# uingei/hevc

Hardware: AMD Instinct MI355X
Metric: encoded 1080p30 frames/sec/GPU; PSNR-Y parity vs libx265 at matched bitrate (higher is better)
Workload: dtype u8; 1 GPU; 1920x1080@30 SDR 8-bit Main, crf 19 capped by VBV maxrate 2940 kbps / bufsize 3528 kbit (the reference's libx265 operating point), 300-frame synthetic 'motion' clip per GPU, keyint 90 (4 closed GOPs of equal length), IPPP, full-search +-15, one clip per GPU, input resident in HBM

## Files before the change

### hevc_amd/csrc/kernels/common.h

```cpp
#pragma once
#include <stdint.h>

#if defined(__HIPCC__)
#include <hip/hip_runtime.h>
#define DEV __device__ __forceinline__
#define HD __host__ __device__
#define HDI __host__ __device__ inline
#define DEVCONST __device__ const
#define MIHEVC_GPU 1
#else
#define DEV inline
#define HD
#define HDI inline
#define DEVCONST static const
#define MIHEVC_GPU 0
#endif

#include "../../../include/mihevc.h"

namespace mihevc {

constexpr int CTU = 32;
constexpr int CTU_LOG2 = 5;
constexpr int PAD_Y = 80;
// ... 58 lines not shown
        for (int n = 0; n < 32; n++) {
            int a = (k * (2 * n + 1)) % 128;
            if (a > 64) a = 128 - a;
            t.mat[k][n] = (int8_t)(a > 32 ? -c64[64 - a] : c64[a]);
        }
    const int d[4][4] = {{29, 55, 74, 84}, {74, 74, 0, -74}, {84, -29, -74, 55}, {55, -84, 74, -29}};
    for (int i = 0; i < 4; i++) for (int j = 0; j < 4; j++) t.dst4[i][j] = (int8_t)d[i][j];
    const int lt[4][8] = {{0, 0, 0, 64, 0, 0, 0, 0}, {-1, 4, -10, 58, 17, -5, 1, 0}, {-1, 4, -11, 40, 40, -11, 4, -1}, {0, 1, -5, 17, 58, -10, 4, -1}};
    for (int i = 0; i < 4; i++) for (int j = 0; j < 8; j++) t.luma_tap[i][j] = (int8_t)lt[i][j];
    const int ct[8][4] = {{0, 64, 0, 0}, {-2, 58, 10, -2}, {-4, 54, 16, -2}, {-6, 46, 28, -4}, {-4, 36, 36, -4}, {-4, 28, 46, -6}, {-2, 16, 54, -4}, {-2, 10, 58, -2}};
    for (int i = 0; i < 8; i++) for (int j = 0; j < 4; j++) t.chroma_tap[i][j] = (int8_t)ct[i][j];
    const int ang[35] = {0, 0, 32, 26, 21, 17, 13, 9, 5, 2, 0, -2, -5, -9, -13, -17, -21, -26, -32, -26, -21, -17, -13, -9, -5, -2, 0, 2, 5, 9, 13, 17, 21, 26, 32};
    for (int i = 0; i < 35; i++) t.intra_angle[i] = (int8_t)ang[i];
    const int inv[15] = {-4096, -1638, -910, -630, -482, -390, -315, -256, -315, -390, -482, -630, -910, -1638, -4096};
    for (int i = 0; i < 15; i++) t.inv_angle[i] = (int16_t)inv[i];
    for (int q = 0; q < 52; q++) t.beta[q] = (uint8_t)(q < 16 ? 0 : q < 29 ? q - 10 : 2 * q - 38);
    const int tcv[54] = {0, 0, 0, 0, 0, 0, 0, 0, 0, 0, 0, 0, 0, 0, 0, 0, 0, 0, 1, 1, 1, 1, 1, 1, 1, 1, 1, 2, 2, 2, 2, 3, 3, 3, 3, 4, 4, 4,
                         5, 5, 6, 6, 7, 8, 9, 10, 11, 13, 14, 16, 18, 20, 22, 24};
    for (int i = 0; i < 54; i++) t.tc[i] = (uint8_t)tcv[i];
    const int qs[6] = {26214, 23302, 20560, 18396, 16384, 14564}, ls[6] = {40, 45, 51, 57, 64, 72};
    for (int i = 0; i < 6; i++) { t.quant_scale[i] = (int16_t)qs[i]; t.level_scale[i] = (uint8_t)ls[i]; }
    const int cq[14] = {29, 30, 31, 32, 33, 33, 34, 34, 35, 35, 36, 36, 37, 37};
    for (int i = 0; i < 14; i++) t.chroma_qp[i] = (int8_t)cq[i];
    for (int ty = 0; ty < 4; ty++)
        for (int tx = 0; tx < 4; tx++) t.zorder[ty * 4 + tx] = (uint8_t)(((ty >> 1) * 2 + (tx >> 1)) * 4 + (ty & 1) * 2 + (tx & 1));
    return t;
}
DEVCONST Tables g_tab = make_tables();

DEV int iabs(int v) { return v < 0 ? -v : v; }
DEV int imin(int a, int b) { return a < b ? a : b; }
DEV int imax(int a, int b) { return a > b ? a : b; }
DEV int clip3(int lo, int hi, int v) { return v < lo ? lo : v > hi ? hi : v; }
DEV int ilog2u(unsigned v) { return 31 - __builtin_clz(v | 1); }
DEV int mvd_bits(int d)
{
    int a = iabs(d);
    return a == 0 ? 1 : a == 1 ? 3 : 3 + 2 * ilog2u((unsigned)a);
}
DEV int chroma_qp_of(int qp)
{
    int q = clip3(-12, 57, qp);
    return q < 30 ? q : q > 43 ? q - 6 : g_tab.chroma_qp[q - 30];
}
DEV int zaddr(int x, int y, int ctus_w)
{
    int bx = (x & 31) >> 2, by = (y & 31) >> 2, z = 0;
    for (int i = 0; i < 3; i++) z |= ((bx >> i) & 1) << (2 * i) | ((by >> i) & 1) << (2 * i + 1);
    return (((y >> CTU_LOG2) * ctus_w + (x >> CTU_LOG2)) << 6) | z;
}
DEV void node_geom(int node, int &x, int &y, int &log2n)
{
    if (node == 0) { x = 0; y = 0; log2n = 5; }
    else if (node < 5) { int q = node - 1; x = (q & 1) * 16; y = (q >> 1) * 16; log2n = 4; }
    else { int q = (node - 5) >> 2, s = (node - 5) & 3; x = (q & 1) * 16 + (s & 1) * 8; y = (q >> 1) * 16 + (s >> 1) * 8; log2n = 3; }
}
DEV int node_of_tile(int level, int tx, int ty)
{
    if (level == 0) return 0;
    int q = (ty >> 1) * 2 + (tx >> 1);
    return level == 1 ? 1 + q : 5 + q * 4 + (ty & 1) * 2 + (tx & 1);
}

DEV uint32_t sad_packed_u8(uint32_t a, uint32_t b, uint32_t acc)
{
#if MIHEVC_GPU
    return __builtin_amdgcn_sad_u8(a, b, acc);
#else
    for (int i = 0; i < 4; i++) acc += (uint32_t)iabs((int)((a >> (8 * i)) & 255) - (int)((b >> (8 * i)) & 255));
    return acc;
#endif
}
DEV uint32_t load_u32(const void *p)
{
    uint32_t v;
    __builtin_memcpy(&v, p, 4);
    return v;
}
DEV uint32_t pk_add16(uint32_t a, uint32_t b)
{
#if MIHEVC_GPU
    typedef short v2s __attribute__((ext_vector_type(2)));
    return __builtin_bit_cast(uint32_t, (v2s)(__builtin_bit_cast(v2s, a) + __builtin_bit_cast(v2s, b)));
#else
    return ((a + b) & 0xffffu) | (((a >> 16) + (b >> 16)) << 16);
#endif
}
DEV uint32_t pk_sub16(uint32_t a, uint32_t b)
{
#if MIHEVC_GPU
    typedef short v2s __attribute__((ext_vector_type(2)));
    return __builtin_bit_cast(uint32_t, (v2s)(__builtin_bit_cast(v2s, a) - __builtin_bit_cast(v2s, b)));
#else
    return ((a - b) & 0xffffu) | (((a >> 16) - (b >> 16)) << 16);
#endif
}
DEV uint32_t pk_max_i16(uint32_t a, uint32_t b)
{
#if MIHEVC_GPU
    uint32_t r;
    asm("v_pk_max_i16 %0, %1, %2" : "=v"(r) : "v"(a), "v"(b));
    return r;
#else
    const int al = (int16_t)(a & 0xffffu), ah = (int16_t)(a >> 16), bl = (int16_t)(b & 0xffffu), bh = (int16_t)(b >> 16);
    return (uint32_t)((al > bl ? al : bl) & 0xffff) | ((uint32_t)((ah > bh ? ah : bh) & 0xffff) << 16);
#endif
}

DEV uint32_t perm_bytes(uint32_t a, uint32_t b, uint32_t sel)
{
#if MIHEVC_GPU
    return __builtin_amdgcn_perm(a, b, sel);
#else
    const uint64_t ab = ((uint64_t)a << 32) | b;
    uint32_t r = 0;
    for (int i = 0; i < 4; i++) r |= (uint32_t)((ab >> (8 * ((sel >> (8 * i)) & 7))) & 255u) << (8 * i);
    return r;
#endif
}
DEV void transpose_bytes4(const uint32_t (&r)[4], uint32_t (&c)[4])
{
    const uint32_t t0 = perm_bytes(r[1], r[0], 0x05010400u), t1 = perm_bytes(r[1], r[0], 0x07030602u);
    const uint32_t t2 = perm_bytes(r[3], r[2], 0x05010400u), t3 = perm_bytes(r[3], r[2], 0x07030602u);
    c[0] = perm_bytes(t2, t0, 0x05040100u); c[1] = perm_bytes(t2, t0, 0x07060302u);
    c[2] = perm_bytes(t3, t1, 0x05040100u); c[3] = perm_bytes(t3, t1, 0x07060302u);
}

#if !MIHEVC_GPU
inline bool g_emu_mixed_wave = false;
#endif
DEV bool wave_all(bool p)
{
#if MIHEVC_GPU
    return __all(p) != 0;
#else
    return p && !g_emu_mixed_wave;
#endif
}

DEV uint64_t qsad_u8(uint64_t ref8, uint32_t cur, uint64_t acc)
{
#if MIHEVC_GPU
    return __builtin_amdgcn_qsad_pk_u16_u8(ref8, cur, acc);
#else
    uint64_t out = 0;
    for (int j = 0; j < 4; j++) {
        uint32_t w = (uint32_t)(ref8 >> (8 * j)), a = (uint32_t)((acc >> (16 * j)) & 0xffff);
        for (int i = 0; i < 4; i++) a += (uint32_t)iabs((int)((w >> (8 * i)) & 255) - (int)((cur >> (8 * i)) & 255));
        out |= (uint64_t)(a & 0xffff) << (16 * j);
    }
    return out;
#endif
}
DEV uint32_t align_bytes(uint32_t hi, uint32_t lo, int shift_bytes)
{
#if MIHEVC_GPU
    return __builtin_amdgcn_alignbyte(hi, lo, (uint32_t)shift_bytes);
#else
    return (uint32_t)(((((uint64_t)hi) << 32) | lo) >> (8 * shift_bytes));
#endif
}
template <typename T>
DEV void copy_window(T *lds, int ls, const T *plane, int pstride, int ox, int oy, int w, int h, int lo_x, int hi_x, int lo_y, int hi_y, int tid)
{
    constexpr int per = 4 / (int)sizeof(T);
    constexpr int CH = 6;
    const int dpr = w / per, col = tid & 31, rg = tid >> 5;
    for (int d = col; d < dpr; d += 32) {
        const int x = clip3(lo_x, hi_x - (per - 1), ox + d * per);
        for (int r0 = rg; r0 < h; r0 += CH * (NT / 32)) {
            uint32_t v[CH];
#pragma unroll
            for (int k = 0; k < CH; k++) {
                const int r = r0 + k * (NT / 32);
                if (r < h) v[k] = load_u32(plane + (ptrdiff_t)clip3(lo_y, hi_y, oy + r) * pstride + x);
            }
#pragma unroll
            for (int k = 0; k < CH; k++) {
                const int r = r0 + k * (NT / 32);
                if (r < h) __builtin_memcpy(__builtin_assume_aligned(lds + r * ls + d * per, 4), &v[k], 4);
            }
        }
    }
}

DEV int wave_uniform(int v)
{
#if MIHEVC_GPU
    v = __builtin_amdgcn_readfirstlane(v);
#endif
    return v;
}
DEV int opaque_zero()
{
    int z = 0;
#if MIHEVC_GPU
    asm volatile("" : "+v"(z));
#endif
    return z;
}
DEV uint32_t load_u32_aligned(const void *p)
{
    uint32_t v;
    __builtin_memcpy(&v, __builtin_assume_aligned(p, 4), 4);
    return v;
}
DEV void store_u32_aligned(void *p, uint32_t v) { __builtin_memcpy(__builtin_assume_aligned(p, 4), &v, 4); }
DEV void store4(uint8_t *p, int v0, int v1, int v2, int v3) { store_u32_aligned(p, (uint32_t)v0 | (uint32_t)v1 << 8 | (uint32_t)v2 << 16 | (uint32_t)v3 << 24); }
DEV void store4(uint16_t *p, int v0, int v1, int v2, int v3)
{
    store_u32_aligned(p, (uint32_t)v0 | (uint32_t)v1 << 16);
    store_u32_aligned(p + 2, (uint32_t)v2 | (uint32_t)v3 << 16);
}
DEV void store4(int16_t *p, int v0, int v1, int v2, int v3)
{
    store_u32_aligned(p, ((uint32_t)v0 & 0xffffu) | (uint32_t)v1 << 16);
    store_u32_aligned(p + 2, ((uint32_t)v2 & 0xffffu) | (uint32_t)v3 << 16);
}
DEV void load_row8(const uint8_t *base, int idx, int (&px)[8])
{
    const int off = idx & 3;
    const uint8_t *p = base + (idx - off);
    const uint32_t d0 = load_u32_aligned(p), d1 = load_u32_aligned(p + 4), d2 = load_u32_aligned(p + 8);
    const uint32_t r0 = align_bytes(d1, d0, off), r1 = align_bytes(d2, d1, off);
#pragma unroll
    for (int i = 0; i < 4; i++) { px[i] = (int)((r0 >> (8 * i)) & 255); px[4 + i] = (int)((r1 >> (8 * i)) & 255); }
}
DEV void load_row8(const uint16_t *base, int idx, int (&px)[8])
{
    const int off = idx & 1;
    const uint16_t *p = base + (idx - off);
    uint32_t d[5];
#pragma unroll
    for (int k = 0; k < 5; k++) d[k] = load_u32_aligned(p + 2 * k);
#pragma unroll
    for (int k = 0; k < 4; k++) {
        const uint32_t r = align_bytes(d[k + 1], d[k], 2 * off);
        px[2 * k] = (int)(r & 65535); px[2 * k + 1] = (int)(r >> 16);
    }
}

DEV int dot4_i8(uint32_t a, uint32_t b, int acc)
{
#if MIHEVC_GPU
    return __builtin_amdgcn_sdot4((int)a, (int)b, acc, false);
#else
    for (int i = 0; i < 4; i++) acc += (int)(int8_t)(a >> (8 * i)) * (int)(int8_t)(b >> (8 * i));
    return acc;
#endif
}
DEV int dot2_i16(uint32_t a, uint32_t b, int acc)
{
#if MIHEVC_GPU
    typedef short v2s __attribute__((ext_vector_type(2)));
    v2s va, vb;
    __builtin_memcpy(&va, &a, 4);
    __builtin_memcpy(&vb, &b, 4);
    return __builtin_amdgcn_sdot2(va, vb, acc, false);
#else
    return acc + (int)(int16_t)(a & 0xffff) * (int)(int16_t)(b & 0xffff) + (int)(int16_t)(a >> 16) * (int)(int16_t)(b >> 16);
#endif
}
DEV int dot4_i8_start(uint32_t a, uint32_t b, int start)
{
#if MIHEVC_GPU
    return __builtin_amdgcn_sdot4((int)a, (int)b, start, true);
#else
    return dot4_i8(a, b, start);
#endif
}
DEV int dot2_i16_start(uint32_t a, uint32_t b, int start)
{
#if MIHEVC_GPU
    typedef short v2s __attribute__((ext_vector_type(2)));
    v2s va, vb;
    __builtin_memcpy(&va, &a, 4);
    __builtin_memcpy(&vb, &b, 4);
    return __builtin_amdgcn_sdot2(va, vb, start, true);
#else
    return dot2_i16(a, b, start);
#endif
}

DEV uint32_t pack_lo16(int lo, int hi)
{
#if MIHEVC_GPU
    return __builtin_amdgcn_perm((uint32_t)hi, (uint32_t)lo, 0x05040100u);
#else
    return ((uint32_t)lo & 0xffffu) | ((uint32_t)hi << 16);
#endif
}

DEV void butterfly8(int (&d)[8])
{
#pragma unroll
    for (int st = 1; st < 8; st <<= 1)
#pragma unroll
        for (int i = 0; i < 8; i++)
            if (!(i & st)) { int p = d[i], q = d[i + st]; d[i] = p + q; d[i + st] = p - q; }
}
template <bool AC> DEV int hadamard8_sum(int (&m)[8][8])
{
#pragma unroll
    for (int y = 0; y < 8; y++) butterfly8(m[y]);
    int s = 0;
#pragma unroll
    for (int x = 0; x < 8; x++) {
#pragma unroll
        for (int st = 1; st < 8; st <<= 1)
#pragma unroll
            for (int i = 0; i < 8; i++)
                if (!(i & st)) { int p = m[i][x], q = m[i + st][x]; m[i][x] = p + q; m[i + st][x] = p - q; }
#pragma unroll
        for (int i = 0; i < 8; i++) if (!AC || x || i) s += iabs(m[i][x]);
    }
    return (s + 2) >> 2;
}
DEV int hadamard8_satd(int (&m)[8][8]) { return hadamard8_sum<false>(m); }
DEV int hadamard8_ac(int (&m)[8][8]) { return hadamard8_sum<true>(m); }

typedef uint32_t mfma_frag __attribute__((vector_size(16), may_alias));
typedef float mfma_acc __attribute__((vector_size(16)));
DEV float half_bits_to_float(uint32_t h)
{
#if MIHEVC_GPU && defined(__HIP_DEVICE_COMPILE__)
    const uint16_t b16 = (uint16_t)h;
    _Float16 v;
    __builtin_memcpy(&v, &b16, 2);
    return (float)v;
#else
    const uint32_t e = (h >> 10) & 31u, m = h & 1023u, b = e == 31 ? 0x7f800000u | m << 13 : (e + 112u) << 23 | m << 13;
    float f;
    __builtin_memcpy(&f, &b, 4);
    const float mag = e == 0 ? (float)(int)m * 0x1p-24f : f;
    return (h & 0x8000u) ? -mag : mag;
#endif
}
#if MIHEVC_GPU
#ifdef MIHEVC_PHASE_PROF
__device__ unsigned long long g_phase_prof[8 * 1024 * 3];
#endif
struct GpuExec {
    static DEV int lane_id()
    {
        int t = (int)threadIdx.x;
        asm volatile("" : "+v"(t));
        return t;
    }
#ifdef MIHEVC_PHASE_PROF
    template <class F> DEV void phase(F &&f, int line = __builtin_LINE(), const char *file = __builtin_FILE())
    {
        int len = 0;
// ... 140 lines not shown
```

### hevc_amd/csrc/kernels/inter.h

```cpp
#pragma once
#include "common.h"
#include "residual.h"

namespace mihevc {

template <typename T> struct InterArgs {
    Plane<const T> src[3];
    Plane<const T> ref[3];
    Plane<T> rec[3];
    int w, h, ctus_w;
    CostParams prm;
    const int16_t *centers;
    int32_t *me;
    mihevc_cu_rec *cu;
    int16_t *coef[3];
    unsigned long long *est;
    int sparse_coef;
    IpInfo *ip;
    Plane<const T> ref1[3];
    const int16_t *centers1;
    int32_t *me1;
};
template <typename T> DEV InterArgs<T> list1_view(const InterArgs<T> &a)
{
    InterArgs<T> b = a;
    for (int i = 0; i < 3; i++) b.ref[i] = a.ref1[i];
    b.centers = a.centers1; b.me = a.me1;
    return b;
}

DEVCONST int8_t kOff[9][2] = {{0, 0}, {-1, -1}, {0, -1}, {1, -1}, {-1, 0}, {1, 0}, {-1, 1}, {0, 1}, {1, 1}};
DEVCONST int8_t kRingSlot[8] = {4, 5, 2, 7, 1, 3, 6, 8};

template <typename T> struct PreArgs {
    Plane<const T> src, ref;
    uint8_t *lsrc, *lref;
    int w, h, bit_depth;
    int16_t *centers;
    unsigned *cost;
};
template <typename T> DEV void lowres_sample(const PreArgs<T> &a, int i)
{
    const int lw = a.w >> 2, n = lw * (a.h >> 2), sh = a.bit_depth - 8;
    if (i >= 2 * n) return;
    const Plane<const T> &p = i < n ? a.src : a.ref;
    const int k = i < n ? i : i - n, x = k % lw, y = k / lw;
    int s = 8 << sh;
#pragma unroll
    for (int j = 0; j < 4; j++) {
        const T *row = p.p + (ptrdiff_t)(4 * y + j) * p.stride + 4 * x;
        if (sizeof(T) == 1) {
            s = (int)sad_packed_u8(load_u32(row), 0u, (uint32_t)s);
        } else
            s += (int)row[0] + (int)row[1] + (int)row[2] + (int)row[3];
    }
    s >>= 4 + sh;
    (i < n ? a.lsrc : a.lref)[k] = (uint8_t)(s < 255 ? s : 255);
}
constexpr int PRE_SPAN = 2 * PRE_RANGE + 1;
constexpr int PRE_WIN_W = 40;
constexpr int PRE_WIN_STRIDE = 96;
struct PreShared {
    uint8_t blk[64];
    uint8_t win[(8 + 2 * PRE_RANGE) * PRE_WIN_STRIDE + 16];
    unsigned long long best;
    unsigned sad0;
};
template <typename T, class Ex> DEV void pre_search_program(Ex &ex, PreShared &s, const PreArgs<T> &a, int ctu)
{
    constexpr int R = PRE_RANGE, span = PRE_SPAN;
    const int lw = a.w >> 2, lh = a.h >> 2, wc = (lw + 7) >> 3, cx = ctu % wc, cy = ctu / wc;
    const int bw = lw - 8 * cx < 8 ? lw - 8 * cx : 8, bh = lh - 8 * cy < 8 ? lh - 8 * cy : 8;
    ex.phase([&](int tid) {
        if (tid < 64) { const int x = tid & 7, y = tid >> 3; s.blk[tid] = (x < bw && y < bh) ? a.lsrc[(8 * cy + y) * lw + 8 * cx + x] : (uint8_t)0; }
        if (8 * cx - R >= 0 && 8 * cx - R + PRE_WIN_W <= lw && 8 * cy - R >= 0 && 8 * cy + 8 + R <= lh) {
            constexpr int DPR = PRE_WIN_W / 4, ND = (8 + 2 * PRE_RANGE) * DPR, IT = (ND + NT - 1) / NT;
            uint32_t v[IT];
#pragma unroll
            for (int k = 0; k < IT; k++) {
                const int i = tid + k * NT;
                if (i < ND) v[k] = load_u32(a.lref + (size_t)(8 * cy - R + i / DPR) * lw + 8 * cx - R + 4 * (i % DPR));
            }
#pragma unroll
            for (int k = 0; k < IT; k++) {
                const int i = tid + k * NT;
                if (i < ND) store_u32_aligned(s.win + (i / DPR) * PRE_WIN_STRIDE + 4 * (i % DPR), v[k]);
            }
        } else {
            constexpr int NW = (8 + 2 * PRE_RANGE) * PRE_WIN_W, IT = (NW + NT - 1) / NT;
            uint8_t v[IT];
#pragma unroll
            for (int k = 0; k < IT; k++) {
                const int i = tid + k * NT;
                if (i < NW) v[k] = a.lref[clip3(0, lh - 1, 8 * cy + i / PRE_WIN_W - R) * lw + clip3(0, lw - 1, 8 * cx + i % PRE_WIN_W - R)];
            }
#pragma unroll
            for (int k = 0; k < IT; k++) {
                const int i = tid + k * NT;
                if (i < NW) s.win[(i / PRE_WIN_W) * PRE_WIN_STRIDE + i % PRE_WIN_W] = v[k];
            }
        }
        if (tid == 0) s.best = ~0ull;
    });
    ex.phase([&](int tid) {
        unsigned long long best = ~0ull;
        if (bw == 8 && bh == 8) {
            if (tid < 8 * span) {
                const int q = tid & 7, dyi = tid >> 3;
                uint64_t acc = 0;
#pragma unroll
                for (int y = 0; y < 8; y++) {
                    const uint8_t *w = s.win + (y + dyi) * PRE_WIN_STRIDE + 4 * q;
                    const uint32_t r0 = load_u32_aligned(w), r1 = load_u32_aligned(w + 4), r2 = load_u32_aligned(w + 8);
                    acc = qsad_u8(((uint64_t)r1 << 32) | r0, load_u32_aligned(s.blk + 8 * y), acc);
                    acc = qsad_u8(((uint64_t)r2 << 32) | r1, load_u32_aligned(s.blk + 8 * y + 4), acc);
                }
#pragma unroll
                for (int j = 0; j < 4; j++) {
                    const int dxi = 4 * q + j;
                    if (dxi >= span) continue;
                    const unsigned sad = (unsigned)((acc >> (16 * j)) & 0xffff);
                    if (dxi == R && dyi == R) s.sad0 = sad;
                    const unsigned long long key = ((unsigned long long)(4 * sad + (unsigned)(iabs(dxi - R) + iabs(dyi - R))) << 12) | (unsigned)(dyi * span + dxi);
                    best = key < best ? key : best;
                }
            }
        } else {
            for (int p = tid; p < span * span; p += NT) {
                const int dxi = p % span, dyi = p / span;
                unsigned sad = 0;
                for (int y = 0; y < bh; y++)
                    for (int x = 0; x < bw; x++) sad += (unsigned)iabs((int)s.blk[y * 8 + x] - (int)s.win[(y + dyi) * PRE_WIN_STRIDE + x + dxi]);
                if (dxi == R && dyi == R) s.sad0 = sad;
                const unsigned long long key = ((unsigned long long)(4 * sad + (unsigned)(iabs(dxi - R) + iabs(dyi - R))) << 12) | (unsigned)p;
                best = key < best ? key : best;
            }
        }
        if (best != ~0ull) ex.atomic_min(&s.best, best);
    });
    ex.phase([&](int tid) {
        if (tid != 0) return;
        int p = (int)(s.best & 4095);
        const unsigned sad_best = (unsigned)(((s.best >> 12) - (unsigned)(iabs(p % span - R) + iabs(p / span - R))) >> 2);
        if (2 * sad_best >= s.sad0) p = R * span + R;
        a.centers[2 * ctu] = (int16_t)(4 * (p % span - R));
        a.centers[2 * ctu + 1] = (int16_t)(4 * (p / span - R));
        if (a.cost) a.cost[ctu] = sad_best;
    });
}

DEV bool mv_rows_ok(int y, int n, int my, int h, int top, int bottom)
{
    const int ly0 = y + (my >> 2) - ((my & 3) ? 3 : 0), ly1 = y + n - 1 + (my >> 2) + ((my & 3) ? 4 : 0);
    const int cy0 = (y >> 1) + (my >> 3) - ((my & 7) ? 1 : 0), cy1 = (y >> 1) + (n >> 1) - 1 + (my >> 3) + ((my & 7) ? 2 : 0);
    if (top && (ly0 < 0 || cy0 < 0)) return false;
    if (bottom && (ly1 > h - 1 || cy1 > (h >> 1) - 1)) return false;
    return true;
}
DEV int clamp_center_y(int sy, int y0, int R, int h, int top, int bottom)
{
    const int ctu_h = h - y0 < CTU ? h - y0 : CTU;
    if (bottom && sy > h - (y0 + ctu_h) - R) sy = h - (y0 + ctu_h) - R;
    if (top && sy < R - y0) sy = R - y0;
    return sy;
}

template <typename T> struct MeShared {
    uint8_t src[32 * 32];
    unsigned long long best[21];
    uint8_t valid[21];
    unsigned nodeok[2 * MAX_RANGE + 1];
};
HDI int me_spanx(int R) { return ((2 * R + 1) + 3) & ~3; }
HDI int me_win_w(int R) { return 32 + me_spanx(R); }
HDI int me_win_stride(int R)
{
    int u = (me_win_w(R) + 4 + 3) >> 2;
    while ((u & 15) != 8) u++;
    return u << 2;
}
HDI int me_win_elems(int R) { return (32 + 2 * R) * me_win_stride(R) + 16; }

template <int ROWS> DEV void quad_block_row(const uint8_t *src, const uint8_t *ref, int ws, unsigned (&out)[4][4])
{
    uint64_t acc[4] = {0, 0, 0, 0};
#pragma unroll(ROWS)
    for (int r = 0; r < 8; r++) {
        uint32_t rr[9], cc[8];
#pragma unroll
        for (int d = 0; d < 9; d++) rr[d] = load_u32_aligned(ref + r * ws + 4 * d);
#pragma unroll
        for (int d = 0; d < 8; d++) cc[d] = load_u32_aligned(src + r * 32 + 4 * d);
#pragma unroll
        for (int d = 0; d < 8; d++) acc[d >> 1] = qsad_u8(((uint64_t)rr[d + 1] << 32) | rr[d], cc[d], acc[d >> 1]);
    }
#pragma unroll
    for (int b = 0; b < 4; b++)
#pragma unroll
        for (int j = 0; j < 4; j++) out[b][j] = (unsigned)((acc[b] >> (16 * j)) & 0xffff);
}
DEV void copy_window_msb(uint8_t *lds, int ls, const uint16_t *plane, int pstride, int ox, int oy, int w, int h, int lo_x, int hi_x, int lo_y, int hi_y, int sh, int tid)
{
    const int dpr = w / 4, col = tid & 31, rg = tid >> 5;
    for (int r = rg; r < h; r += NT / 32) {
        const int y = clip3(lo_y, hi_y, oy + r);
        const uint16_t *srow = plane + (ptrdiff_t)y * pstride;
        for (int d = col; d < dpr; d += 32) {
            const int x = clip3(lo_x, hi_x - 3, ox + d * 4);
            const uint32_t a = load_u32(srow + x), b = load_u32(srow + x + 2);
            const uint32_t v = ((a & 0xffffu) >> sh) | (((a >> 16) >> sh) << 8) | (((b & 0xffffu) >> sh) << 16) | (((b >> 16) >> sh) << 24);
            store_u32_aligned(lds + r * ls + d * 4, v);
        }
    }
}
DEV void copy_window_msb(uint8_t *lds, int ls, const uint8_t *plane, int pstride, int ox, int oy, int w, int h, int lo_x, int hi_x, int lo_y, int hi_y, int, int tid)
{
    copy_window<uint8_t>(lds, ls, plane, pstride, ox, oy, w, h, lo_x, hi_x, lo_y, hi_y, tid);
}

template <typename T, int RANGE = 0, class Ex>
DEV void me_search_program(Ex &ex, MeShared<T> &s, uint8_t *win, const InterArgs<T> &a, int ctu)
{
    const int msb = sizeof(T) == 1 ? 0 : a.prm.bit_depth - 8;

    const int R = RANGE ? RANGE : a.prm.me_range, spany = 2 * R + 1, spanx = me_spanx(R), quads = spanx >> 2, ws = me_win_stride(R), ww = me_win_w(R), wh = 32 + 2 * R;
    const int x0 = (ctu % a.ctus_w) * CTU, y0 = (ctu / a.ctus_w) * CTU;
    const int mct = a.prm.mc_top, mcb = a.prm.mc_bottom;
    const int sx = wave_uniform(a.centers ? a.centers[2 * ctu] : 0), sy0 = wave_uniform(a.centers ? a.centers[2 * ctu + 1] : 0);
    const int sy = (mct || mcb) ? clamp_center_y(sy0, y0, R, a.h, mct, mcb) : sy0;
    ex.phase([&](int tid) {
        if (sizeof(T) == 1 && x0 + CTU <= a.w && y0 + CTU <= a.h) {
            const uint32_t v = load_u32(a.src[0].p + (size_t)(y0 + (tid >> 3)) * a.src[0].stride + x0 + 4 * (tid & 7));
            store_u32_aligned(s.src + 4 * tid, v);
        } else
        for (int i = tid; i < 1024; i += NT) {
            int x = x0 + (i & 31), y = y0 + (i >> 5);
            s.src[i] = (x < a.w && y < a.h) ? (uint8_t)(a.src[0].p[(size_t)y * a.src[0].stride + x] >> msb) : (uint8_t)0;
        }
        copy_window_msb(win, ws, a.ref[0].p, a.ref[0].stride, x0 + sx - R, y0 + sy - R, ww, wh, -PAD_Y, a.w + PAD_Y - 1, -PAD_Y, a.h + PAD_Y - 1, msb, tid);
        if (tid < 21) {
            int nx, ny, nl;
            node_geom(tid, nx, ny, nl);
            s.valid[tid] = x0 + nx + (1 << nl) <= a.w && y0 + ny + (1 << nl) <= a.h;
            s.best[tid] = ~0ull;
        }
        for (int dyi = tid; dyi < spany; dyi += NT) {
            unsigned bits = 0;
            for (int n = 0; n < 21; n++) {
                int nx, ny, nl;
                node_geom(n, nx, ny, nl);
                const bool in_pic = x0 + nx + (1 << nl) <= a.w && y0 + ny + (1 << nl) <= a.h;
                if (in_pic && (!(mct || mcb) || mv_rows_ok(y0 + ny, 1 << nl, 4 * (sy + dyi - R), a.h, mct, mcb))) bits |= 1u << n;
            }
            s.nodeok[dyi] = bits;
        }
    });
    ex.phase([&](int tid) {
#ifdef MIHEVC_EXP_DPP_MIN
        for (int it0 = 0; it0 < quads * spany; it0 += NT) {
            const int item = it0 + tid < quads * spany ? it0 + tid : 0;
            const int q = item % quads, dyi = item / quads;
            const unsigned ok = it0 + tid < quads * spany ? s.nodeok[dyi] : 0u, pos0 = (unsigned)(dyi * spanx + 4 * q);
#else
        for (int item = tid; item < quads * spany; item += NT) {
            const int q = item % quads, dyi = item / quads;
            const unsigned ok = s.nodeok[dyi], pos0 = (unsigned)(dyi * spanx + 4 * q);
#endif
            const int by = mvd_bits(4 * (dyi - R)), ksh = 6 + msb;
            const uint8_t *srcp = s.src + opaque_zero();
            unsigned bitsj[4], s32[4] = {0, 0, 0, 0};
#pragma unroll
            for (int j = 0; j < 4; j++) bitsj[j] = ((unsigned)(a.prm.lambda_sad_q4 * (mvd_bits(4 * (4 * q + j - R)) + by)) << 2) | (unsigned)j;
            auto consider = [&](int node, const unsigned (&sad)[4]) {
                unsigned k = (sad[0] << ksh) + bitsj[0];
#pragma unroll
                for (int j = 1; j < 4; j++) { const unsigned kj = (sad[j] << ksh) + bitsj[j]; k = kj < k ? kj : k; }
#ifdef MIHEVC_EXP_DPP_MIN
                unsigned long long key = ((ok >> node) & 1) ? (((unsigned long long)(k >> 2) << 16) | (pos0 + (k & 3))) : ~0ull;
                auto step = [&](auto ctrl, auto row_mask) {
                    const unsigned lo = (unsigned)key, hi = (unsigned)(key >> 32);
                    const unsigned tl = (unsigned)__builtin_amdgcn_update_dpp((int)lo, (int)lo, decltype(ctrl)::value, decltype(row_mask)::value, 0xf, false);
                    const unsigned th = (unsigned)__builtin_amdgcn_update_dpp((int)hi, (int)hi, decltype(ctrl)::value, decltype(row_mask)::value, 0xf, false);
                    const unsigned long long t = ((unsigned long long)th << 32) | tl;
                    key = t < key ? t : key;
                };
                step(std::integral_constant<int, 0x111>{}, std::integral_constant<int, 0xf>{});
                step(std::integral_constant<int, 0x112>{}, std::integral_constant<int, 0xf>{});
                step(std::integral_constant<int, 0x114>{}, std::integral_constant<int, 0xf>{});
                step(std::integral_constant<int, 0x118>{}, std::integral_constant<int, 0xf>{});
                step(std::integral_constant<int, 0x142>{}, std::integral_constant<int, 0xa>{});
                step(std::integral_constant<int, 0x143>{}, std::integral_constant<int, 0xc>{});
                if ((tid & 63) == 63 && key < ex.peek(&s.best[node])) ex.atomic_min(&s.best[node], key);
#else
                if (!((ok >> node) & 1)) return;
                const unsigned long long key = ((unsigned long long)(k >> 2) << 16) | (pos0 + (k & 3));
                if (key < ex.peek(&s.best[node])) ex.atomic_min(&s.best[node], key);
#endif
            };
#pragma unroll
            for (int half = 0; half < 2; half++) {
                unsigned s16[2][4] = {{0, 0, 0, 0}, {0, 0, 0, 0}};
#pragma unroll
                for (int r2 = 0; r2 < 2; r2++) {
                    const int br = half * 2 + r2;
                    unsigned o[4][4];
                    quad_block_row<(RANGE ? 4 : 2)>(srcp + br * 8 * 32, win + (br * 8 + dyi) * ws + 4 * q, ws, o);
#pragma unroll
                    for (int b = 0; b < 4; b++) {
#pragma unroll
                        for (int j = 0; j < 4; j++) s16[b >> 1][j] += o[b][j];
                        consider(5 + (half * 2 + (b >> 1)) * 4 + r2 * 2 + (b & 1), o[b]);
                    }
                }
#pragma unroll
                for (int h2 = 0; h2 < 2; h2++) {
#pragma unroll
                    for (int j = 0; j < 4; j++) s32[j] += s16[h2][j];
                    consider(1 + half * 2 + h2, s16[h2]);
                }
            }
            consider(0, s32);
        }
    });
    ex.phase([&](int tid) {
        if (tid < 21) {
            int32_t *o = a.me + ((size_t)ctu * 21 + tid) * 3;
            if (s.valid[tid]) {
                int p = (int)(s.best[tid] & 0xffff);
                o[0] = 4 * (sx + p % spanx - R); o[1] = 4 * (sy + p / spanx - R); o[2] = (int32_t)(s.best[tid] >> 16);
            } else { o[0] = 0; o[1] = 0; o[2] = -1; }
        }
    });
}

template <typename T> struct InterShared {
    ResidualShared rs;
    T src[1536];
    T pred[1536];
    int mvx[21], mvy[21];
    unsigned cost[21];
    uint8_t valid[21];
    int satd[3][1][16];
    unsigned nsum[21];
    unsigned fsum[8][21];
    unsigned long long rbest[21];
    unsigned j16[4];
    int use16[4], use32;
    uint8_t alias[3][16];
    int tile_mvx[16], tile_mvy[16];
    uint8_t tile_node[16];
    uint8_t chosen[21];
    unsigned est;
    unsigned ip_cost, ip_act, ip_tiles;
    unsigned long long ip_sse;
    unsigned tu_dc[3][16], tu_dz[3][16], tu_bits[3][16], tu_zero[3];
};
constexpr int FRAC_PAIR_SUM = 8 * NT;
constexpr int FRAC_SCRATCH = FRAC_PAIR_SUM + NT;
static_assert(FRAC_SCRATCH <= (int)(sizeof(ResidualShared::scratch) / 4), "the fractional search's exchange must fit rs.scratch");
HDI constexpr int mc_win_y(int R) { return (32 + 2 * (R + 3) + 8 + 3) & ~3; }
HDI constexpr int mc_win_y_stride(int R) { return mc_win_y(R) + 4; }
HDI constexpr bool mc_win_y_rows_dword_aligned()
{
    for (int R = 0; R <= MAX_RANGE; R++)
        if (mc_win_y_stride(R) % 4 != 0) return false;
    return true;
}
static_assert(mc_win_y_rows_dword_aligned(), "mc_win_y_stride must be a multiple of 4 samples");
HDI int mc_win_c(int R) { return (16 + (R + 3) + 8 + 3) & ~3; }
HDI int mc_win_c_stride(int R) { return mc_win_c(R) + 4; }
template <typename T> HDI size_t mc_win_y_bytes(int R) { return ((size_t)mc_win_y(R) * mc_win_y_stride(R) + 16) * sizeof(T); }
template <typename T> HDI size_t mc_win_c_bytes(int R) { return ((size_t)mc_win_c(R) * mc_win_c_stride(R) + 16) * sizeof(T); }
HDI constexpr size_t align16(size_t v) { return (v + 15) & ~(size_t)15; }

struct BiShared {
    int mx0[21], my0[21];
    unsigned c0[21], cb[21];
    uint8_t mode[21];
    uint8_t tile_mode[16];
    int tile_mv1x[16], tile_mv1y[16];
    alignas(16) int16_t p0[1536];
};

struct InterLds { size_t y, u, v, bytes; };
template <typename T> HDI constexpr size_t inter_win_in() { return offsetof(InterShared<T>, rs) + offsetof(ResidualShared, scratch) + 4 * (size_t)FRAC_SCRATCH; }
template <typename T> HDI constexpr size_t inter_win_out() { return align16(sizeof(InterShared<T>)); }
template <typename T> HDI InterLds inter_lds(int R)
{
    const size_t n[3] = {mc_win_y_bytes<T>(R), mc_win_c_bytes<T>(R), mc_win_c_bytes<T>(R)};
    const size_t hi = offsetof(InterShared<T>, rs) + offsetof(ResidualShared, scratch) + sizeof(ResidualShared::scratch);
    size_t in = inter_win_in<T>(), out = inter_win_out<T>(), at[3];
    for (int i = 0; i < 3; i++) {
        const size_t r = align16(n[i]);
        if (in + r <= hi) { at[i] = in; in += r; } else { at[i] = out; out += r; }
    }
    return InterLds{at[0], at[1], at[2], out};
}
struct InterBLds { size_t y, u, v, bi, bytes; };
template <typename T> HDI InterBLds inter_b_lds(int R)
{
    InterBLds l;
    l.y = inter_win_out<T>();
    l.u = l.y + align16(mc_win_y_bytes<T>(R));
    l.v = l.u + align16(mc_win_c_bytes<T>(R));
    l.bi = l.v + align16(mc_win_c_bytes<T>(R));
    l.bytes = l.bi + align16(sizeof(BiShared));
    return l;
}

struct TapBytes { uint32_t lo, hi; };
struct TapPairs { uint32_t p[4]; };
DEV TapBytes tap_bytes(int f) { return TapBytes{load_u32(&g_tab.luma_tap[f][0]), load_u32(&g_tab.luma_tap[f][4])}; }
DEV TapPairs tap_pairs(int f)
{
    TapPairs t;
#pragma unroll
    for (int k = 0; k < 4; k++) t.p[k] = pack_lo16(g_tab.luma_tap[f][2 * k], g_tab.luma_tap[f][2 * k + 1]);
    return t;
}
template <typename T> DEV auto row_taps(int f)
{
    if constexpr (sizeof(T) == 1) return tap_bytes(f); else return tap_pairs(f);
}

constexpr int LUMA_ROW_BIAS = 128 * 64;
DEV void luma_row4_at(const uint8_t *p, int off, const TapBytes &t, int, int (&hv)[4])
{
    uint32_t d[4], q[3];
#pragma unroll
    for (int k = 0; k < 4; k++) d[k] = load_u32_aligned(p + 4 * k);
#pragma unroll
    for (int k = 0; k < 3; k++) q[k] = align_bytes(d[k + 1], d[k], off) ^ 0x80808080u;
    hv[0] = dot4_i8(q[0], t.lo, dot4_i8_start(q[1], t.hi, 0));
#pragma unroll
    for (int i = 1; i < 4; i++) hv[i] = dot4_i8(align_bytes(q[1], q[0], i), t.lo, dot4_i8_start(align_bytes(q[2], q[1], i), t.hi, 0));
}
DEV void luma_row4_at(const uint16_t *p, int off, const TapPairs &t, int shift1, int (&hv)[4])
{
    uint32_t d[7], e[6], o[5];
#pragma unroll
    for (int k = 0; k < 7; k++) d[k] = load_u32_aligned(p + 2 * k);
#pragma unroll
    for (int k = 0; k < 6; k++) e[k] = align_bytes(d[k + 1], d[k], 2 * off);
#pragma unroll
    for (int k = 0; k < 5; k++) o[k] = align_bytes(e[k + 1], e[k], 2);
#pragma unroll
    for (int i = 0; i < 4; i++) {
        int v = dot2_i16_start((i & 1) ? o[i >> 1] : e[i >> 1], t.p[0], 0);
#pragma unroll
        for (int k = 1; k < 4; k++) v = dot2_i16((i & 1) ? o[(i >> 1) + k] : e[(i >> 1) + k], t.p[k], v);
        hv[i] = v >> shift1;
    }
}
template <typename T> constexpr int luma_row_bias() { return sizeof(T) == 1 ? LUMA_ROW_BIAS : 0; }
template <typename T> DEV int dword_offset(int idx) { return idx & (4 / (int)sizeof(T) - 1); }

template <typename T> DEV void luma_quad14(const T *win, int i00, int ws, int fx, int fy, int bit_depth, int (&out)[4])
{
    const auto tx = row_taps<T>(fx);
    const int8_t *ty = g_tab.luma_tap[fy];
    const int idx = i00 - 3 * ws - 3, off = dword_offset<T>(idx);
    int acc[4];
#pragma unroll
    for (int i = 0; i < 4; i++) acc[i] = 64 * luma_row_bias<T>();
#pragma unroll
    for (int r = 0; r < 8; r++) {
        int hv[4];
        luma_row4_at(win + (idx - off) + r * ws, off, tx, bit_depth - 8, hv);
        const int t = ty[r];
#pragma unroll
        for (int i = 0; i < 4; i++) acc[i] += t * hv[i];
    }
#pragma unroll
    for (int i = 0; i < 4; i++) out[i] = acc[i] >> 6;
}
template <typename T> DEV int chroma_sample14(const T *p00, int ws, int fx, int fy, int bit_depth)
// ... 677 lines not shown
```

Measured before the change: 6605 frames/s.

## Restructure ME SAD search to share ref rows across dy pairs and split CTU halves

Reworks the full-search ME inner loop so each thread handles two vertically adjacent search offsets, reusing each loaded reference row for both via a held source row. Each CTU is split into top and bottom halves across paired lanes, whose 32x32 sums are exchanged through LDS. Per-x and per-y lambda cost keys are precomputed into LDS tables, and v_mad_u32_u16 with op_sel forms the cost keys. The aim is fewer LDS reference loads and less per-candidate cost arithmetic, at the price of more registers, an extra wave-chain exchange and a changed window stride and size.

```diff
diff --git a/hevc_amd/csrc/kernels/common.h b/hevc_amd/csrc/kernels/common.h
--- a/hevc_amd/csrc/kernels/common.h
+++ b/hevc_amd/csrc/kernels/common.h
@@ -234,6 +234,17 @@
     return out;
 #endif
 }
+template <bool HI> DEV uint32_t mad_field_u16(uint32_t v, uint32_t m, uint32_t add)
+{
+#if MIHEVC_GPU && defined(__HIP_DEVICE_COMPILE__)
+    uint32_t d;
+    if (HI) asm("v_mad_u32_u16 %0, %1, %2, %3 op_sel:[1,0,0,0]" : "=v"(d) : "v"(v), "v"(m), "v"(add));
+    else asm("v_mad_u32_u16 %0, %1, %2, %3" : "=v"(d) : "v"(v), "v"(m), "v"(add));
+    return d;
+#else
+    return ((HI ? v >> 16 : v & 0xffffu) * (m & 0xffffu)) + add;
+#endif
+}
 DEV uint32_t align_bytes(uint32_t hi, uint32_t lo, int shift_bytes)
 {
 #if MIHEVC_GPU
@@ -280,6 +291,13 @@
     asm volatile("" : "+v"(z));
 #endif
     return z;
+}
+DEV int opaque(int v)
+{
+#if MIHEVC_GPU
+    asm volatile("" : "+v"(v));
+#endif
+    return v;
 }
 DEV uint32_t load_u32_aligned(const void *p)
 {
diff --git a/hevc_amd/csrc/kernels/inter.h b/hevc_amd/csrc/kernels/inter.h
--- a/hevc_amd/csrc/kernels/inter.h
+++ b/hevc_amd/csrc/kernels/inter.h
@@ -169,36 +169,51 @@
     uint8_t src[32 * 32];
     unsigned long long best[21];
     uint8_t valid[21];
-    unsigned nodeok[2 * MAX_RANGE + 1];
+    alignas(16) uint32_t xkey[(2 * MAX_RANGE + 1 + 3) & ~3];
+    struct Dy { uint32_t key, barred; };
+    alignas(16) Dy ykey[2 * MAX_RANGE + 2];
+    alignas(16) uint32_t xch[NT / 2][8];
 };
 HDI int me_spanx(int R) { return ((2 * R + 1) + 3) & ~3; }
 HDI int me_win_w(int R) { return 32 + me_spanx(R); }
 HDI int me_win_stride(int R)
 {
     int u = (me_win_w(R) + 4 + 3) >> 2;
-    while ((u & 15) != 8) u++;
+    while ((u & 7) != 4) u++;
     return u << 2;
 }
-HDI int me_win_elems(int R) { return (32 + 2 * R) * me_win_stride(R) + 16; }
-
-template <int ROWS> DEV void quad_block_row(const uint8_t *src, const uint8_t *ref, int ws, unsigned (&out)[4][4])
-{
-    uint64_t acc[4] = {0, 0, 0, 0};
-#pragma unroll(ROWS)
-    for (int r = 0; r < 8; r++) {
-        uint32_t rr[9], cc[8];
-#pragma unroll
-        for (int d = 0; d < 9; d++) rr[d] = load_u32_aligned(ref + r * ws + 4 * d);
-#pragma unroll
-        for (int d = 0; d < 8; d++) cc[d] = load_u32_aligned(src + r * 32 + 4 * d);
-#pragma unroll
-        for (int d = 0; d < 8; d++) acc[d >> 1] = qsad_u8(((uint64_t)rr[d + 1] << 32) | rr[d], cc[d], acc[d >> 1]);
-    }
-#pragma unroll
-    for (int b = 0; b < 4; b++)
-#pragma unroll
-        for (int j = 0; j < 4; j++) out[b][j] = (unsigned)((acc[b] >> (16 * j)) & 0xffff);
-}
+HDI int me_win_elems(int R) { return (33 + 2 * R) * me_win_stride(R) + 16; }
+
+template <bool A, bool B> DEV void quad_row_pair(const uint8_t *ref, const uint8_t *src, uint32_t (&held)[8], uint64_t (&acc_a)[4], uint64_t (&acc_b)[4])
+{
+    uint32_t rr[9], cc[8];
+#pragma unroll
+    for (int d = 0; d < 9; d++) rr[d] = load_u32_aligned(ref + 4 * d);
+    if (A) {
+#pragma unroll
+        for (int d = 0; d < 8; d++) cc[d] = load_u32_aligned(src + 4 * d);
+    }
+#pragma unroll
+    for (int d = 0; d < 8; d++) {
+        const uint64_t pair = ((uint64_t)rr[d + 1] << 32) | rr[d];
+        if (B) acc_b[d >> 1] = qsad_u8(pair, held[d], acc_b[d >> 1]);
+        if (A) acc_a[d >> 1] = qsad_u8(pair, cc[d], acc_a[d >> 1]);
+    }
+    if (A) {
+#pragma unroll
+        for (int d = 0; d < 8; d++) held[d] = cc[d];
+    }
+}
+DEV void settle(uint64_t (&acc_a)[4], uint64_t (&acc_b)[4])
+{
+#if MIHEVC_GPU
+#pragma unroll
+    for (int i = 0; i < 4; i++) asm volatile("" : "+v"(acc_a[i]), "+v"(acc_b[i]));
+#endif
+}
+struct MeHalfSums { uint32_t v[2][4]; };
+static_assert(((1024ull * 255) << (4 + 2)) + (1093ull << 2) * 38 < (1ull << 28), "a search cost and its 3-bit index must fit 31 bits");
+static_assert((2 * MAX_RANGE + 1) * (((2 * MAX_RANGE + 1) + 3) & ~3) < 65536, "a search position must fit the key's 16 bits");
 DEV void copy_window_msb(uint8_t *lds, int ls, const uint16_t *plane, int pstride, int ox, int oy, int w, int h, int lo_x, int hi_x, int lo_y, int hi_y, int sh, int tid)
 {
     const int dpr = w / 4, col = tid & 31, rg = tid >> 5;
@@ -227,7 +242,7 @@
     const int x0 = (ctu % a.ctus_w) * CTU, y0 = (ctu / a.ctus_w) * CTU;
     const int mct = a.prm.mc_top, mcb = a.prm.mc_bottom;
     const int sx = wave_uniform(a.centers ? a.centers[2 * ctu] : 0), sy0 = wave_uniform(a.centers ? a.centers[2 * ctu + 1] : 0);
-    const int sy = (mct || mcb) ? clamp_center_y(sy0, y0, R, a.h, mct, mcb) : sy0;
+    const int sy = wave_uniform((mct || mcb) ? clamp_center_y(sy0, y0, R, a.h, mct, mcb) : sy0);
     ex.phase([&](int tid) {
         if (sizeof(T) == 1 && x0 + CTU <= a.w && y0 + CTU <= a.h) {
             const uint32_t v = load_u32(a.src[0].p + (size_t)(y0 + (tid >> 3)) * a.src[0].stride + x0 + 4 * (tid & 7));
@@ -244,84 +259,137 @@
             s.valid[tid] = x0 + nx + (1 << nl) <= a.w && y0 + ny + (1 << nl) <= a.h;
             s.best[tid] = ~0ull;
         }
-        for (int dyi = tid; dyi < spany; dyi += NT) {
+        for (int dyi = tid; dyi <= spany; dyi += NT) {
             unsigned bits = 0;
-            for (int n = 0; n < 21; n++) {
+            for (int n = 0; n < 21 && dyi < spany; n++) {
                 int nx, ny, nl;
                 node_geom(n, nx, ny, nl);
                 const bool in_pic = x0 + nx + (1 << nl) <= a.w && y0 + ny + (1 << nl) <= a.h;
                 if (in_pic && (!(mct || mcb) || mv_rows_ok(y0 + ny, 1 << nl, 4 * (sy + dyi - R), a.h, mct, mcb))) bits |= 1u << n;
             }
-            s.nodeok[dyi] = bits;
-        }
-    });
-    ex.phase([&](int tid) {
-#ifdef MIHEVC_EXP_DPP_MIN
-        for (int it0 = 0; it0 < quads * spany; it0 += NT) {
-            const int item = it0 + tid < quads * spany ? it0 + tid : 0;
-            const int q = item % quads, dyi = item / quads;
-            const unsigned ok = it0 + tid < quads * spany ? s.nodeok[dyi] : 0u, pos0 = (unsigned)(dyi * spanx + 4 * q);
-#else
-        for (int item = tid; item < quads * spany; item += NT) {
-            const int q = item % quads, dyi = item / quads;
-            const unsigned ok = s.nodeok[dyi], pos0 = (unsigned)(dyi * spanx + 4 * q);
-#endif
-            const int by = mvd_bits(4 * (dyi - R)), ksh = 6 + msb;
-            const uint8_t *srcp = s.src + opaque_zero();
-            unsigned bitsj[4], s32[4] = {0, 0, 0, 0};
-#pragma unroll
-            for (int j = 0; j < 4; j++) bitsj[j] = ((unsigned)(a.prm.lambda_sad_q4 * (mvd_bits(4 * (4 * q + j - R)) + by)) << 2) | (unsigned)j;
-            auto consider = [&](int node, const unsigned (&sad)[4]) {
-                unsigned k = (sad[0] << ksh) + bitsj[0];
-#pragma unroll
-                for (int j = 1; j < 4; j++) { const unsigned kj = (sad[j] << ksh) + bitsj[j]; k = kj < k ? kj : k; }
-#ifdef MIHEVC_EXP_DPP_MIN
-                unsigned long long key = ((ok >> node) & 1) ? (((unsigned long long)(k >> 2) << 16) | (pos0 + (k & 3))) : ~0ull;
-                auto step = [&](auto ctrl, auto row_mask) {
-                    const unsigned lo = (unsigned)key, hi = (unsigned)(key >> 32);
-                    const unsigned tl = (unsigned)__builtin_amdgcn_update_dpp((int)lo, (int)lo, decltype(ctrl)::value, decltype(row_mask)::value, 0xf, false);
-                    const unsigned th = (unsigned)__builtin_amdgcn_update_dpp((int)hi, (int)hi, decltype(ctrl)::value, decltype(row_mask)::value, 0xf, false);
-                    const unsigned long long t = ((unsigned long long)th << 32) | tl;
-                    key = t < key ? t : key;
-                };
-                step(std::integral_constant<int, 0x111>{}, std::integral_constant<int, 0xf>{});
-                step(std::integral_constant<int, 0x112>{}, std::integral_constant<int, 0xf>{});
-                step(std::integral_constant<int, 0x114>{}, std::integral_constant<int, 0xf>{});
-                step(std::integral_constant<int, 0x118>{}, std::integral_constant<int, 0xf>{});
-                step(std::integral_constant<int, 0x142>{}, std::integral_constant<int, 0xa>{});
-                step(std::integral_constant<int, 0x143>{}, std::integral_constant<int, 0xc>{});
-                if ((tid & 63) == 63 && key < ex.peek(&s.best[node])) ex.atomic_min(&s.best[node], key);
-#else
-                if (!((ok >> node) & 1)) return;
-                const unsigned long long key = ((unsigned long long)(k >> 2) << 16) | (pos0 + (k & 3));
-                if (key < ex.peek(&s.best[node])) ex.atomic_min(&s.best[node], key);
-#endif
+            s.ykey[dyi].key = ((unsigned)(a.prm.lambda_sad_q4 * mvd_bits(4 * (dyi - R))) << 3) | (unsigned)((dyi & 1) << 2);
+            s.ykey[dyi].barred = ~bits;
+        }
+        for (int dxi = tid; dxi < spanx; dxi += NT) s.xkey[dxi] = ((unsigned)(a.prm.lambda_sad_q4 * mvd_bits(4 * (dxi - R))) << 3) | (unsigned)(dxi & 3);
+    });
+    const int units = quads * ((spany + 1) >> 1), ksh = 7 + msb;
+    struct Item { int half, q, dy0; };
+    auto item_of = [&](int tid, int u0) {
+        const int unit = u0 + (tid >> 6) * 32 + (tid & 31);
+        return unit < units ? (unit % quads) | (2 * (unit / quads)) << 8 | ((tid >> 5) & 1) << 16 : -1;
+    };
+    auto slot_of = [](int tid) { return (tid >> 6) * 32 + (tid & 31); };
+    auto unpack = [](int item) { return Item{(item >> 16) & 1, item & 255, (item >> 8) & 255}; };
+    auto fresh = [&](int item) { return unpack(RANGE ? item : opaque(item)); };
+    struct Keys { uint32_t x[4], y[4]; };
+    auto keys_of = [&](const Item &it) {
+        Keys k;
+        load_x4(s.xkey + 4 * it.q, k.x);
+        load_x4(s.ykey + it.dy0, k.y);
+        return k;
+    };
+    auto field = [](uint64_t v, int j) { return (unsigned)((v >> (16 * j)) & 0xffff); };
+    auto rank8 = [&](const Keys &k, const unsigned (&sad)[2][4], int node_shift, int node) {
+        unsigned r[2];
+#pragma unroll
+        for (int e = 0; e < 2; e++) {
+            r[e] = (sad[e][0] << ksh) + k.x[0];
+#pragma unroll
+            for (int j = 1; j < 4; j++) { const unsigned kj = (sad[e][j] << ksh) + k.x[j]; r[e] = kj < r[e] ? kj : r[e]; }
+            r[e] = (r[e] + k.y[2 * e]) | (unsigned)((int)((k.y[2 * e + 1] >> node_shift) << (31 - node)) >> 31);
+        }
+        return r[1] < r[0] ? r[1] : r[0];
+    };
+    auto rank4 = [&](const Keys &k, uint64_t sad, int e, int node_shift, int node) {
+        const uint32_t lo = (uint32_t)sad, hi = (uint32_t)(sad >> 32), m = 1u << ksh;
+        const unsigned r0 = mad_field_u16<false>(lo, m, k.x[0]), r1 = mad_field_u16<true>(lo, m, k.x[1]), r2 = mad_field_u16<false>(hi, m, k.x[2]), r3 = mad_field_u16<true>(hi, m, k.x[3]);
+        const unsigned a = r1 < r0 ? r1 : r0, b = r3 < r2 ? r3 : r2, r = b < a ? b : a;
+        return (r + k.y[2 * e]) | (unsigned)((int)((k.y[2 * e + 1] >> node_shift) << (31 - node)) >> 31);
+    };
+    auto bid = [&](unsigned long long *best, unsigned k, const Item &it) {
+        if (k == ~0u) return;
+        const unsigned pos = (unsigned)(it.dy0 * spanx + 4 * it.q) + ((k & 4) ? (unsigned)spanx : 0u) + (k & 3);
+        const unsigned long long key = ((unsigned long long)(k >> 3) << 16) | pos;
+        if (key < ex.peek(best)) ex.atomic_min(best, key);
+    };
+    for (int u0 = 0; u0 < units; u0 += NT / 2) {
+        wave_chain(ex, [&](int tid) -> MeHalfSums {
+            MeHalfSums sums{};
+            const int item = item_of(tid, u0);
+            if (item < 0) return sums;
+            const Item it = unpack(item);
+            const uint8_t *srcp = s.src + 512 * it.half + opaque_zero();
+            uint64_t acc_a[4] = {0, 0, 0, 0}, acc_b[4] = {0, 0, 0, 0};
+            uint64_t s16[2][2] = {{0, 0}, {0, 0}};
+            uint32_t held[8];
+            unsigned ka[4];
+            auto end_a = [&](int r2) __attribute__((always_inline)) {
+                const Item it = fresh(item);
+                const Keys k = keys_of(it);
+#pragma unroll
+                for (int b = 0; b < 4; b++) {
+                    ka[b] = rank4(k, acc_a[b], 0, 8 * it.half, 5 + (b >> 1) * 4 + r2 * 2 + (b & 1));
+                    s16[0][b >> 1] += acc_a[b];
+                    acc_a[b] = 0;
+                }
             };
-#pragma unroll
-            for (int half = 0; half < 2; half++) {
-                unsigned s16[2][4] = {{0, 0, 0, 0}, {0, 0, 0, 0}};
-#pragma unroll
-                for (int r2 = 0; r2 < 2; r2++) {
-                    const int br = half * 2 + r2;
-                    unsigned o[4][4];
-                    quad_block_row<(RANGE ? 4 : 2)>(srcp + br * 8 * 32, win + (br * 8 + dyi) * ws + 4 * q, ws, o);
-#pragma unroll
-                    for (int b = 0; b < 4; b++) {
-#pragma unroll
-                        for (int j = 0; j < 4; j++) s16[b >> 1][j] += o[b][j];
-                        consider(5 + (half * 2 + (b >> 1)) * 4 + r2 * 2 + (b & 1), o[b]);
-                    }
+            auto end_b = [&](int r2) __attribute__((always_inline)) {
+                const Item it = fresh(item);
+                const Keys k = keys_of(it);
+#pragma unroll
+                for (int b = 0; b < 4; b++) {
+                    const int node = 5 + (b >> 1) * 4 + r2 * 2 + (b & 1);
+                    const unsigned kb = rank4(k, acc_b[b], 1, 8 * it.half, node);
+                    bid(s.best + 8 * it.half + node, kb < ka[b] ? kb : ka[b], it);
+                    s16[1][b >> 1] += acc_b[b];
+                    acc_b[b] = 0;
                 }
-#pragma unroll
-                for (int h2 = 0; h2 < 2; h2++) {
-#pragma unroll
-                    for (int j = 0; j < 4; j++) s32[j] += s16[h2][j];
-                    consider(1 + half * 2 + h2, s16[h2]);
-                }
-            }
-            consider(0, s32);
-        }
-    });
+            };
+            const uint8_t *ref = win + (16 * it.half + it.dy0) * ws + 4 * it.q;
+            quad_row_pair<true, false>(ref, srcp, held, acc_a, acc_b);
+            settle(acc_a, acc_b);
+#pragma unroll
+            for (int r = 1; r < 16; r++) {
+                quad_row_pair<true, true>(ref + r * ws, srcp + r * 32, held, acc_a, acc_b);
+                if (r == 7 || r == 15) end_a(r >> 3);
+                if (r == 8) end_b(0);
+                settle(acc_a, acc_b);
+            }
+            quad_row_pair<false, true>(ref + 16 * ws, srcp, held, acc_a, acc_b);
+            end_b(1);
+            const Item at = fresh(item);
+            const Keys k = keys_of(at);
+#pragma unroll
+            for (int h2 = 0; h2 < 2; h2++)
+            {
+                const unsigned k0 = rank4(k, s16[0][h2], 0, 2 * at.half, 1 + h2), k1 = rank4(k, s16[1][h2], 1, 2 * at.half, 1 + h2);
+                bid(s.best + 2 * at.half + 1 + h2, k1 < k0 ? k1 : k0, at);
+            }
+#pragma unroll
+            for (int e = 0; e < 2; e++)
+#pragma unroll
+                for (int j = 0; j < 4; j++) sums.v[e][j] = field(s16[e][0], j) + field(s16[e][1], j);
+            if (at.half) {
+                store_x4(s.xch[slot_of(tid)], sums.v[0]);
+                store_x4(s.xch[slot_of(tid)] + 4, sums.v[1]);
+            }
+            return sums;
+        }, [&](int tid, const MeHalfSums &sums) {
+            const int item = item_of(tid, u0);
+            if (item < 0 || (item >> 16)) return;
+            const Item it = unpack(item);
+            uint32_t low[2][4];
+            load_x4(s.xch[slot_of(tid)], low[0]);
+            load_x4(s.xch[slot_of(tid)] + 4, low[1]);
+            unsigned sad[2][4];
+#pragma unroll
+            for (int e = 0; e < 2; e++)
+#pragma unroll
+                for (int j = 0; j < 4; j++) sad[e][j] = sums.v[e][j] + low[e][j];
+            bid(s.best, rank8(keys_of(it), sad, 0, 0), it);
+        });
+    }
+    ex.phase([](int) {});
     ex.phase([&](int tid) {
         if (tid < 21) {
             int32_t *o = a.me + ((size_t)ctu * 21 + tid) * 3;
```

After: 6521 frames/s. 0.987x the previous value.
